# joshuacwnewton/swiftwatcher

Measured on AMD Instinct MI355X. Metric: frames/sec (segment+classify) on 1080p ROI batches, higher is better.
Workload: dtype f64 (image_filtering), f32 (CNN)

## Files before the change

include/swk.h:

```cpp
#ifndef SWK_H
#define SWK_H

#include <stdint.h>

#ifdef __cplusplus
extern "C" {
#endif

#define SWK_ABI_VERSION 2

enum {
    SWK_OK = 0,
    SWK_ERR_ARG = -1,
    SWK_ERR_HIP = -2,
    SWK_ERR_NOGPU = -3,
    SWK_ERR_CAPACITY = -4,
    SWK_ERR_NOMEM = -5,
    SWK_ERR_STALE = -6
};

enum { SWK_MEM_HOST = 0, SWK_MEM_DEVICE = 1 };

enum { SWK_ORDER_RASTER = 0, SWK_ORDER_BLOCK2X2 = 1 };

// ... 106 lines not shown
int32_t swk_regionprops_u8(swk_ctx *ctx, const uint8_t *labels, int32_t count, int32_t H, int32_t W,
                           int32_t seg_cap, swk_segment *segs, int32_t *nseg);

int32_t swk_classifier_input(swk_ctx *ctx, const uint8_t *crops, int64_t crops_bytes, const int64_t *offsets,
                             const int32_t *hw, int32_t nseg, const float mean[3], const float std_[3],
                             uint8_t *patches, float *net, int32_t net_mem);
int32_t swk_classifier_input_window(swk_ctx *ctx, const uint8_t *crops, int64_t crops_bytes, const int64_t *offsets,
                                    const int32_t *hw, int32_t nseg, const float mean[3], const float std_[3],
                                    int32_t pad, int32_t channels_last, uint8_t *patches, float *net, int32_t net_mem);

int32_t swk_segment_inputs(swk_ctx *ctx, const swk_input *in, int32_t frame_h, int32_t frame_w,
                           const swk_segment *segs, const int32_t *nseg, int32_t seg_cap, int32_t min_h, int32_t min_w,
                           const float mean[3], const float std_[3], int32_t pad, int32_t channels_last, int32_t first,
                           int32_t net_cap, float *net, int32_t *seg_frame, int32_t *total, int32_t *skipped);
int32_t swk_segment_inputs_last(swk_ctx *ctx, int32_t min_h, int32_t min_w, const float mean[3], const float std_[3],
                                int32_t pad, int32_t channels_last, int32_t first, int32_t net_cap, float *net,
                                int32_t *seg_frame, int32_t *total, int32_t *skipped);

int32_t swk_nhwc_bias_relu_place(void *stream, const float *src, int32_t n, int32_t sh, int32_t sw, int32_t c, int32_t crop_y,
                                 int32_t crop_x, int32_t h, int32_t w, const float *bias, float *dst, int32_t dH, int32_t dW,
                                 int32_t dC, int32_t off_y, int32_t off_x, int32_t c_off);
int32_t swk_nhwc_maxpool3s2(void *stream, const float *src, int32_t n, int32_t h, int32_t w, int32_t c, float *dst);
int32_t swk_nhwc_head2_relu_mean(void *stream, const float *x, int32_t n, int32_t px, int32_t c, const float *w, const float *bias,
                                 const float *ring, float n_pos, float *out);
int32_t swk_nhwc_head2_dropout_relu_mean(void *stream, const float *x, int32_t n, int32_t px, int32_t c, const int32_t *pos, const float *bg,
                                         int32_t n_pos, const float *w, const float *bias, const uint64_t *keys, uint64_t seed,
                                         int32_t samples, float *out);
int32_t swk_nhwc_conv7x7s2_bias_relu(void *stream, const float *src, int32_t n, int32_t side, int32_t lo, int32_t m, const float *weight,
                                     const float *bias, int32_t cout, float *dst);
int32_t swk_nhwc_conv1x1_bias_relu_place(void *stream, const float *src, int32_t n, int32_t sh, int32_t sw, int32_t cin, int32_t crop_y,
                                         int32_t crop_x, int32_t h, int32_t w, const float *weight, const float *bias, int32_t cout,
                                         float *dst, int32_t dH, int32_t dW, int32_t dC, int32_t off_y, int32_t off_x, int32_t c_off);

int32_t swk_nhwc_maxpool3s2_conv1x1_bias_relu_place(void *stream, const float *src, int32_t n, int32_t t, int32_t cin, const float *weight,
                                                    const float *bias, int32_t cout, float *dst, int32_t dH, int32_t dW, int32_t dC,
                                                    int32_t off_y, int32_t off_x, const float *ring, int32_t live_lo, int32_t live_n);


int32_t swk_nhwc_conv3x3_bias_relu_place(void *stream, const float *src, int32_t n, int32_t t, int32_t cin, const float *weight_t,
                                         const float *bias, int32_t cout, float *dst, int32_t dH, int32_t dW, int32_t dC, int32_t off_y,
                                         int32_t off_x, int32_t c_off);

int32_t swk_winograd_f2x2_3x3_weights(const float *weight, int32_t cout, int32_t cin, float *out);
int32_t swk_nhwc_conv3x3_winograd_bias_relu_place(void *stream, const float *src, int32_t n, int32_t t, int32_t cin, const float *weight_w,
                                                  const float *bias, int32_t cout, float *dst, int32_t dH, int32_t dW, int32_t dC,
                                                  int32_t off_y, int32_t off_x, int32_t c_off);

int32_t swk_winograd_f2x2_3x3_weights_bf16s(const float *weight, int32_t cout, int32_t cin, uint16_t *out);
int32_t swk_nhwc_conv3x3_winograd_bf16s_bias_relu_place(void *stream, const float *src, int32_t n, int32_t t, int32_t cin,
                                                        const uint16_t *weight_s, const float *bias, int32_t cout, float *dst, int32_t dH,
                                                        int32_t dW, int32_t dC, int32_t off_y, int32_t off_x, int32_t c_off);

int32_t swk_track_costs(const double *prev_c, const double *prev_hist0, const uint8_t *prev_has_hist,
                        const double *curr_c, int32_t n_prev, int32_t n_curr, double *cost);
int32_t swk_lsap(const double *cost, int32_t n_rows, int32_t n_cols, int32_t *col4row);

int32_t swk_median_blur_u8(const uint8_t *src, int32_t H, int32_t W, int32_t channels, int32_t ksize, uint8_t *dst);
int32_t swk_otsu_threshold_u8(const uint8_t *src, int64_t count, uint8_t *dst, int32_t *thresh);
int32_t swk_canny_u8(const uint8_t *src, int32_t H, int32_t W, int32_t low, int32_t high, uint8_t *dst);
int32_t swk_dilate_up_u8(const uint8_t *src, int32_t H, int32_t W, int32_t N, uint8_t *dst);
int32_t swk_roi_mask(const uint8_t *frame, int32_t H, int32_t W, int64_t row_stride, const int32_t corners[4],
                     int32_t crop_region[4], uint8_t *mask, int64_t mask_capacity);


#ifdef __cplusplus
}
// ... 3 lines not shown
```

swiftwatcher_amd/_lib.py:

```python
import ctypes
import os
import threading

import numpy as np

_HERE = os.path.dirname(os.path.abspath(__file__))
LIB_PATH = os.environ.get("SWK_LIB", os.path.join(_HERE, "libswk.so"))

ABI_VERSION = 2
MEM_HOST, MEM_DEVICE = 0, 1
ERR_STALE = -6
STAGE_DENSE, STAGE_WHOLE, STAGE_ROWS, STAGE_2D, STAGE_DEVICE = 0, 1, 2, 3, -1
STAGES = ("gray", "rpca", "bilateral", "thresh", "opened", "labels")
ORDER_RASTER, ORDER_BLOCK2X2 = 0, 1
GRAY_Q14, GRAY_Q15 = 0, 1
YUV_I420, YUV_NV12 = 0, 1
K_GRAY, K_IALM_STATS, K_IALM_PASS, K_IALM_SMALL, K_FILTER, K_CCL, K_PROPS, K_COPY = range(8)
KERNEL_FAMILIES = ["gray", "ialm_stats", "ialm_pass", "ialm_small", "filter", "ccl", "props", "copy"]

c_u8p = ctypes.POINTER(ctypes.c_uint8)
c_f64p = ctypes.POINTER(ctypes.c_double)
c_i32p = ctypes.POINTER(ctypes.c_int32)


# ... 66 lines not shown
    "swk_rpca_epilogue": (ctypes.c_int32, [ctypes.c_void_p, ctypes.c_void_p, ctypes.c_int64, ctypes.c_void_p]),
    "swk_bilateral_u8": (ctypes.c_int32, [ctypes.c_void_p, ctypes.c_void_p, ctypes.c_int32, ctypes.c_int32, ctypes.c_int32, ctypes.c_int32, ctypes.c_double, ctypes.c_double, ctypes.c_int32, ctypes.c_void_p]),
    "swk_thresh_tozero_u8": (ctypes.c_int32, [ctypes.c_void_p, ctypes.c_void_p, ctypes.c_int64, ctypes.c_int32, ctypes.c_void_p]),
    "swk_grey_open3x3_u8": (ctypes.c_int32, [ctypes.c_void_p, ctypes.c_void_p, ctypes.c_int32, ctypes.c_int32, ctypes.c_int32, ctypes.c_void_p]),
    "swk_grey_open_u8": (ctypes.c_int32, [ctypes.c_void_p, ctypes.c_void_p] + [ctypes.c_int32] * 5 + [ctypes.c_void_p]),
    "swk_resize_linear_u8": (ctypes.c_int32, [ctypes.c_void_p, ctypes.c_void_p] + [ctypes.c_int32] * 6 + [ctypes.c_void_p]),
    "swk_ccl_u8": (ctypes.c_int32, [ctypes.c_void_p, ctypes.c_void_p, ctypes.c_int32, ctypes.c_int32, ctypes.c_int32, ctypes.c_int32, ctypes.c_int32, ctypes.c_void_p, ctypes.c_void_p]),
    "swk_regionprops_u8": (ctypes.c_int32, [ctypes.c_void_p, ctypes.c_void_p, ctypes.c_int32, ctypes.c_int32, ctypes.c_int32, ctypes.c_int32, ctypes.c_void_p, ctypes.c_void_p]),
    "swk_classifier_input": (ctypes.c_int32, [ctypes.c_void_p, ctypes.c_void_p, ctypes.c_int64, ctypes.c_void_p, ctypes.c_void_p, ctypes.c_int32, ctypes.c_void_p, ctypes.c_void_p, ctypes.c_void_p, ctypes.c_void_p, ctypes.c_int32]),
    "swk_set_sparse_speculation": (ctypes.c_int32, [ctypes.c_void_p, ctypes.c_double]),
    "swk_set_integer_start": (ctypes.c_int32, [ctypes.c_void_p, ctypes.c_int32]),
    "swk_last_integer_start_windows": (ctypes.c_int32, [ctypes.c_void_p, ctypes.c_void_p]),
    "swk_debug_ialm_start": (ctypes.c_int32, [ctypes.c_void_p, ctypes.c_void_p, ctypes.c_int32, ctypes.c_int32, ctypes.c_int32, ctypes.c_double] + [ctypes.c_void_p] * 7),
    "swk_debug_ialm_first_step": (ctypes.c_int32, [ctypes.c_void_p, ctypes.c_void_p, ctypes.c_int32, ctypes.c_int32, ctypes.c_int32, ctypes.c_double] + [ctypes.c_void_p] * 7),
    "swk_last_host_stage": (ctypes.c_int32, [ctypes.c_void_p, ctypes.c_void_p, ctypes.c_int32]),
    "swk_debug_resize_table": (ctypes.c_int32, [ctypes.c_void_p, ctypes.c_int32, ctypes.c_int32, ctypes.c_int32, ctypes.c_void_p, ctypes.c_void_p]),
    "swk_last_eig_sweeps": (ctypes.c_int32, [ctypes.c_void_p, ctypes.c_void_p]),
    "swk_set_norm_speculation": (ctypes.c_int32, [ctypes.c_void_p, ctypes.c_double]),
    "swk_set_norm_guard": (ctypes.c_int32, [ctypes.c_void_p, ctypes.c_double]),
    "swk_prof_guard_windows": (ctypes.c_int32, [ctypes.c_void_p, ctypes.c_void_p]),
    "swk_last_stopping_norms": (ctypes.c_int32, [ctypes.c_void_p, ctypes.c_void_p, ctypes.c_void_p, ctypes.c_int32]),
    "swk_set_start_refine": (ctypes.c_int32, [ctypes.c_void_p, ctypes.c_double]),
    "swk_prof_refined_windows": (ctypes.c_int32, [ctypes.c_void_p, ctypes.c_void_p, ctypes.c_void_p]),
    "swk_prof_pass_bytes_per_element": (ctypes.c_int32, [ctypes.c_void_p, ctypes.c_void_p]),
    "swk_prof_redo_batches": (ctypes.c_int32, [ctypes.c_void_p, ctypes.c_void_p]),
    "swk_prof_redo_windows": (ctypes.c_int32, [ctypes.c_void_p, ctypes.c_void_p]),
    "swk_nhwc_bias_relu_place": (ctypes.c_int32, [ctypes.c_void_p, ctypes.c_void_p] + [ctypes.c_int32] * 8 + [ctypes.c_void_p, ctypes.c_void_p] + [ctypes.c_int32] * 6),
    "swk_set_cnn_tuning": (ctypes.c_int32, [ctypes.c_int32, ctypes.c_int32]),
    "swk_nhwc_conv7x7s2_bias_relu": (ctypes.c_int32, [ctypes.c_void_p, ctypes.c_void_p, ctypes.c_int32, ctypes.c_int32, ctypes.c_int32, ctypes.c_int32, ctypes.c_void_p, ctypes.c_void_p, ctypes.c_int32, ctypes.c_void_p]),
    "swk_nhwc_conv1x1_bias_relu_place": (ctypes.c_int32, [ctypes.c_void_p, ctypes.c_void_p] + [ctypes.c_int32] * 8 + [ctypes.c_void_p, ctypes.c_void_p, ctypes.c_int32, ctypes.c_void_p] + [ctypes.c_int32] * 6),
    "swk_nhwc_conv3x3_bias_relu_place": (ctypes.c_int32, [ctypes.c_void_p, ctypes.c_void_p, ctypes.c_int32, ctypes.c_int32, ctypes.c_int32, ctypes.c_void_p, ctypes.c_void_p, ctypes.c_int32, ctypes.c_void_p] + [ctypes.c_int32] * 6),
    "swk_nhwc_conv3x3_winograd_bias_relu_place": (ctypes.c_int32, [ctypes.c_void_p, ctypes.c_void_p, ctypes.c_int32, ctypes.c_int32, ctypes.c_int32, ctypes.c_void_p, ctypes.c_void_p, ctypes.c_int32, ctypes.c_void_p] + [ctypes.c_int32] * 6),
    "swk_winograd_f2x2_3x3_weights": (ctypes.c_int32, [ctypes.c_void_p, ctypes.c_int32, ctypes.c_int32, ctypes.c_void_p]),
    "swk_nhwc_conv3x3_winograd_bf16s_bias_relu_place": (ctypes.c_int32, [ctypes.c_void_p, ctypes.c_void_p, ctypes.c_int32, ctypes.c_int32, ctypes.c_int32, ctypes.c_void_p, ctypes.c_void_p, ctypes.c_int32, ctypes.c_void_p] + [ctypes.c_int32] * 6),
    "swk_winograd_f2x2_3x3_weights_bf16s": (ctypes.c_int32, [ctypes.c_void_p, ctypes.c_int32, ctypes.c_int32, ctypes.c_void_p]),
    "swk_nhwc_maxpool3s2_conv1x1_bias_relu_place": (ctypes.c_int32, [ctypes.c_void_p, ctypes.c_void_p, ctypes.c_int32, ctypes.c_int32, ctypes.c_int32, ctypes.c_void_p, ctypes.c_void_p, ctypes.c_int32, ctypes.c_void_p] + [ctypes.c_int32] * 5 + [ctypes.c_void_p, ctypes.c_int32, ctypes.c_int32]),
    "swk_nhwc_maxpool3s2": (ctypes.c_int32, [ctypes.c_void_p, ctypes.c_void_p, ctypes.c_int32, ctypes.c_int32, ctypes.c_int32, ctypes.c_int32, ctypes.c_void_p]),
    "swk_nhwc_head2_relu_mean": (ctypes.c_int32, [ctypes.c_void_p, ctypes.c_void_p, ctypes.c_int32, ctypes.c_int32, ctypes.c_int32, ctypes.c_void_p,
                                                  ctypes.c_void_p, ctypes.c_void_p, ctypes.c_float, ctypes.c_void_p]),
    "swk_nhwc_head2_dropout_relu_mean": (ctypes.c_int32, [ctypes.c_void_p, ctypes.c_void_p, ctypes.c_int32, ctypes.c_int32, ctypes.c_int32, ctypes.c_void_p,
                                                          ctypes.c_void_p, ctypes.c_int32, ctypes.c_void_p, ctypes.c_void_p, ctypes.c_void_p, ctypes.c_uint64,
                                                          ctypes.c_int32, ctypes.c_void_p]),
    "swk_segment_inputs": (ctypes.c_int32, [ctypes.c_void_p, ctypes.c_void_p, ctypes.c_int32, ctypes.c_int32, ctypes.c_void_p, ctypes.c_void_p, ctypes.c_int32, ctypes.c_int32, ctypes.c_int32, ctypes.c_void_p, ctypes.c_void_p, ctypes.c_int32, ctypes.c_int32, ctypes.c_int32, ctypes.c_int32, ctypes.c_void_p, ctypes.c_void_p, ctypes.c_void_p, ctypes.c_void_p]),
    "swk_segment_inputs_last": (ctypes.c_int32, [ctypes.c_void_p, ctypes.c_int32, ctypes.c_int32, ctypes.c_void_p, ctypes.c_void_p, ctypes.c_int32, ctypes.c_int32, ctypes.c_int32, ctypes.c_int32, ctypes.c_void_p, ctypes.c_void_p, ctypes.c_void_p, ctypes.c_void_p]),
    "swk_device_alloc": (ctypes.c_int32, [ctypes.c_void_p, ctypes.c_int64, ctypes.POINTER(ctypes.c_void_p)]),
    "swk_device_free": (ctypes.c_int32, [ctypes.c_void_p, ctypes.c_void_p]),
    "swk_device_read": (ctypes.c_int32, [ctypes.c_void_p, ctypes.c_void_p, ctypes.c_void_p, ctypes.c_int64]),
    "swk_classifier_input_window": (ctypes.c_int32, [ctypes.c_void_p, ctypes.c_void_p, ctypes.c_int64, ctypes.c_void_p, ctypes.c_void_p, ctypes.c_int32, ctypes.c_void_p, ctypes.c_void_p, ctypes.c_int32, ctypes.c_int32, ctypes.c_void_p, ctypes.c_void_p, ctypes.c_int32]),
    "swk_track_costs": (ctypes.c_int32, [ctypes.c_void_p, ctypes.c_void_p, ctypes.c_void_p, ctypes.c_void_p, ctypes.c_int32, ctypes.c_int32, ctypes.c_void_p]),
    "swk_lsap": (ctypes.c_int32, [ctypes.c_void_p, ctypes.c_int32, ctypes.c_int32, ctypes.c_void_p]),
    "swk_median_blur_u8": (ctypes.c_int32, [ctypes.c_void_p, ctypes.c_int32, ctypes.c_int32, ctypes.c_int32, ctypes.c_int32, ctypes.c_void_p]),
    "swk_otsu_threshold_u8": (ctypes.c_int32, [ctypes.c_void_p, ctypes.c_int64, ctypes.c_void_p, ctypes.c_void_p]),
    "swk_canny_u8": (ctypes.c_int32, [ctypes.c_void_p, ctypes.c_int32, ctypes.c_int32, ctypes.c_int32, ctypes.c_int32, ctypes.c_void_p]),
    "swk_dilate_up_u8": (ctypes.c_int32, [ctypes.c_void_p, ctypes.c_int32, ctypes.c_int32, ctypes.c_int32, ctypes.c_void_p]),
    "swk_roi_mask": (ctypes.c_int32, [ctypes.c_void_p, ctypes.c_int32, ctypes.c_int32, ctypes.c_int64, ctypes.c_void_p, ctypes.c_void_p, ctypes.c_void_p, ctypes.c_int64]),
    "swk_pinned_alloc": (ctypes.c_int32, [ctypes.c_int32, ctypes.c_int64, ctypes.POINTER(ctypes.c_void_p)]),
    "swk_pinned_free": (ctypes.c_int32, [ctypes.c_void_p]),
    "swk_cut_boxes": (ctypes.c_int32, [ctypes.c_void_p, ctypes.c_int32, ctypes.c_int64, ctypes.c_int32, ctypes.c_int32, ctypes.c_void_p, ctypes.c_void_p, ctypes.c_void_p, ctypes.c_void_p]),
    "swk_stage_frames": (ctypes.c_int32, [ctypes.c_void_p, ctypes.c_int32, ctypes.c_int64, ctypes.c_int32, ctypes.c_int32, ctypes.c_int64, ctypes.c_int64, ctypes.c_void_p, ctypes.c_int32]),
    "swk_prof_enable": (ctypes.c_int32, [ctypes.c_void_p, ctypes.c_int32]),
    "swk_prof_reset": (ctypes.c_int32, [ctypes.c_void_p]),
    "swk_prof_get": (ctypes.c_int32, [ctypes.c_void_p, ctypes.c_int32, ctypes.POINTER(ctypes.c_double), ctypes.POINTER(ctypes.c_int64)]),
    "swk_prof_window_iters": (ctypes.c_int32, [ctypes.c_void_p, ctypes.POINTER(ctypes.c_int64)]),
    "swk_set_ialm_variant": (ctypes.c_int32, [ctypes.c_void_p, ctypes.c_int32]),
    "swk_set_pass_tuning": (ctypes.c_int32, [ctypes.c_void_p, ctypes.c_int32]),
    "swk_set_eig_method": (ctypes.c_int32, [ctypes.c_void_p, ctypes.c_int32]),
# ... 721 lines not shown
```

swiftwatcher_amd/csrc/build.py:

```python
import os
import subprocess
import sys

HERE = os.path.dirname(os.path.abspath(__file__))
PKG = os.path.dirname(HERE)
ROOT = os.path.dirname(PKG)
LIB = os.path.join(PKG, "libswk.so")
SOURCES = ["swk_api.hip", "ialm.hip", "ialm_mfma.hip", "ialm_mstate.hip", "ialm_small.hip", "ialm_refine.hip", "ialm_gram8.hip", "groups.hip", "filters.hip", "yuv.hip", "ccl.hip", "classify_input.hip", "cnn_aux.hip", "cnn_conv1.hip", "cnn_conv1x1.hip", "cnn_expand_bf16.hip", "cnn_conv3x3.hip", "cnn_wino3x3.hip", "cnn_wino3x3_bf16s.hip", "cnn_poolsq.hip", "tracker.cpp", "roi_mask.cpp", "host_stage.cpp"]
HEADERS = ["swk_internal.h", "cnn_common.h", "ialm_small_dev.h", os.path.join(ROOT, "include", "swk.h"), os.path.join(ROOT, "include", "swk_debug.h")]
FLAGS = ["--offload-arch=gfx950", "-O3", "-std=c++17", "-fPIC", "-ffp-contract=off",
         "-fvisibility=hidden", "-Wall", "-Wno-unused-function", "-I", os.path.join(ROOT, "include"), "-I", HERE]


def _stale(out, deps):
    if not os.path.exists(out):
        return True
    t = os.path.getmtime(out)
    return any(os.path.getmtime(d) > t for d in deps)


def build(force=False, verbose=False):
    hipcc = os.environ.get("HIPCC", "/opt/rocm/bin/hipcc")
    objdir = os.path.join(HERE, "build")
    os.makedirs(objdir, exist_ok=True)
    hdrs = [h if os.path.isabs(h) else os.path.join(HERE, h) for h in HEADERS]
    objs = []
    procs = []
    for src in SOURCES:
        sp = os.path.join(HERE, src)
        obj = os.path.join(objdir, src + ".o")
        objs.append(obj)
        if force or _stale(obj, [sp] + hdrs + [os.path.abspath(__file__)]):
            cmd = [hipcc] + FLAGS + ["-c", sp, "-o", obj]
            if verbose:
                print(" ".join(cmd))
            procs.append((src, subprocess.Popen(cmd)))
    for src, p in procs:
        if p.wait() != 0:
            raise RuntimeError("hipcc failed on " + src)
    if force or procs or _stale(LIB, objs):
        cmd = [hipcc, "--offload-arch=gfx950", "-shared", "-fPIC", "-pthread", "-o", LIB] + objs
# ... 9 lines not shown
```

swiftwatcher_amd/csrc/cnn_common.h:

```cpp
#pragma once
#include "swk_internal.h"

#include <cstring>

namespace swk {

typedef float f16v __attribute__((ext_vector_type(16)));
typedef __bf16 bf16x8 __attribute__((ext_vector_type(8)));

struct Place {
    float *dst;
    int dH, dW, dC, off_y, off_x, c_off;
};
struct Crop {
    int sh, sw, crop_y, crop_x;
};

inline bool place_ok(const Place &p, int h, int w, int c, bool quads, const Crop *crop = nullptr)
{
    if (!p.dst || c < 1 || p.off_y < 0 || p.off_x < 0 || p.off_y + h > p.dH || p.off_x + w > p.dW || p.c_off < 0 || p.c_off + c > p.dC) return false;
    if (quads && ((c & 3) || (p.dC & 3) || (p.c_off & 3) || ((uintptr_t)p.dst & 15))) return false;
    return !crop || (crop->crop_y >= 0 && crop->crop_x >= 0 && crop->crop_y + h <= crop->sh && crop->crop_x + w <= crop->sw);
}

int launch_expand1x1_split_bf16(hipStream_t s, const float *src, int64_t rows, const Crop &cr, int cin, int h, int w, const float *wgt,
                                const float *bias, int cout, const Place &pl);
extern int g_expand_split_bf16;
extern int g_wino_bf16s_layout;

__device__ __forceinline__ void store_bias_relu(float *q, const f16v &acc, int g, const float4 b)
{
    float4 v;
    v.x = fmaxf(acc[4 * g] + b.x, 0.0f);
    v.y = fmaxf(acc[4 * g + 1] + b.y, 0.0f);
    v.z = fmaxf(acc[4 * g + 2] + b.z, 0.0f);
    v.w = fmaxf(acc[4 * g + 3] + b.w, 0.0f);
    *(float4 *)q = v;
}

__device__ __forceinline__ void split3(float x, __bf16 &a, __bf16 &b, __bf16 &c)
{
    a = (__bf16)x;
    const float r = x - (float)a;
    b = (__bf16)r;
    c = (__bf16)(r - (float)b);
}
inline void split3_host(float x, uint16_t part[3])
{
    for (int i = 0; i < 3; ++i) {
        uint32_t u;
        float back;
        memcpy(&u, &x, 4);
        u = (u + 0x7fffu + ((u >> 16) & 1u)) & 0xffff0000u;
        memcpy(&back, &u, 4);
        part[i] = (uint16_t)(u >> 16);
        x -= back;
    }
}

inline void winograd_U(const float g[9], double U[4][4])
// ... 31 lines not shown
```

swiftwatcher_amd/csrc/cnn_conv1x1.hip:

```cpp
#include "cnn_common.h"

namespace swk {

template <int NBLK, int KC, int D, int CS, int NWV>
__global__ __launch_bounds__(64 * NWV) void k_conv1x1_relu_place(const float *__restrict__ src, int64_t rows, int sh, int sw, int cin, int crop_y,
                                                            int crop_x, int h, int w, const float *__restrict__ wgt, const float *__restrict__ bias,
                                                            int cout, float *__restrict__ dst, int dH, int dW, int dC, int off_y, int off_x, int c_off,
                                                            FastDiv fhw, FastDiv fw)
{
    constexpr int NP = 32 * NBLK, PITCH = NP + 1, KH = KC / 2, NV = KH / 4, NB = NBLK / CS, NT = 64 * NWV, SLOTS = NWV / CS;
    static_assert(NBLK % CS == 0 && NWV % CS == 0, "column splits");
    extern __shared__ float lds[];
    const int tid = threadIdx.x, lane = tid & 63, wave = tid >> 6, r = lane & 31, hh = lane >> 5;
    float *lbias = lds + ((cin * PITCH + 3) & ~3);
    const int hw = h * w;
    const int cs = wave % CS;
    const int64_t ntiles = (rows + 31) >> 5, stride = (int64_t)gridDim.x * SLOTS;
    int64_t tile = (int64_t)blockIdx.x * SLOTS + wave / CS;

    auto locate = [&](int64_t t, int64_t &ro) -> const float * {
        const unsigned m = (unsigned)t * 32u + (unsigned)r;
        const bool valid = m < (unsigned)rows;
        const unsigned mm = valid ? m : (unsigned)rows - 1u;
        const unsigned b = fhw.div(mm), rem = mm - b * (unsigned)hw;
// ... 140 lines not shown

int32_t swk_nhwc_conv1x1_bias_relu_place(void *stream, const float *src, int32_t n, int32_t sh, int32_t sw, int32_t cin, int32_t crop_y,
                                         int32_t crop_x, int32_t h, int32_t w, const float *weight, const float *bias, int32_t cout,
                                         float *dst, int32_t dH, int32_t dW, int32_t dC, int32_t off_y, int32_t off_x, int32_t c_off)
{
    const swk::Place pl{dst, dH, dW, dC, off_y, off_x, c_off};
    const swk::Crop cr{sh, sw, crop_y, crop_x};
    if (!src || !weight || !bias || n < 1 || h < 1 || w < 1 || cin < 16 || (cin & 15) || cin > 1024 || cout > 256 ||
        !swk::place_ok(pl, h, w, cout, true, &cr) || ((((uintptr_t)src) | ((uintptr_t)weight)) & 15))
        return SWK_ERR_ARG;
    using namespace swk;
    const int64_t rows = (int64_t)n * h * w;
    hipStream_t s = (hipStream_t)stream;
    if (g_expand_split_bf16 && cout == 4 * cin) {
        const int rc = launch_expand1x1_split_bf16(s, src, rows, cr, cin, h, w, weight, bias, cout, pl);
        if (rc != SWK_ERR_ARG) return rc;
    }
    switch ((cout + 31) / 32) {
    case 1: return launch_conv1x1<1>(s, src, rows, cr, cin, h, w, weight, bias, cout, pl);
    case 2: return launch_conv1x1<2>(s, src, rows, cr, cin, h, w, weight, bias, cout, pl);
    case 3: return launch_conv1x1<3>(s, src, rows, cr, cin, h, w, weight, bias, cout, pl);
    case 4: return launch_conv1x1<4>(s, src, rows, cr, cin, h, w, weight, bias, cout, pl);
    case 6: return launch_conv1x1<6>(s, src, rows, cr, cin, h, w, weight, bias, cout, pl);
    case 8: return launch_conv1x1<8>(s, src, rows, cr, cin, h, w, weight, bias, cout, pl);
    default: return SWK_ERR_ARG;
    }
}

int32_t swk_set_cnn_tuning(int32_t knob, int32_t value)
{
    if (knob == 0 && (value == 0 || value == 1)) { swk::g_conv1x1_ring = value; return SWK_OK; }
    if (knob == 1 && (value == 0 || value == 1)) { swk::g_expand_split_bf16 = value; return SWK_OK; }
    if (knob == 2 && value >= 0 && value <= 2) { swk::g_wino_bf16s_layout = value; return SWK_OK; }
    return SWK_ERR_ARG;
}

}
#pragma GCC visibility pop
```

swiftwatcher_amd/segment_classification.py:

```python
import ctypes
import os
import threading

import numpy as np
import torch
from torch import nn

IMAGENET_MEAN = (0.485, 0.456, 0.406)
IMAGENET_STD = (0.229, 0.224, 0.225)
RESIZE = 24
PAD = (224 - 24) // 2


class Fire(nn.Module):

    def __init__(self, inplanes, squeeze_planes, expand1x1_planes, expand3x3_planes):
        super().__init__()
        self.squeeze = nn.Conv2d(inplanes, squeeze_planes, kernel_size=1)
        self.squeeze_activation = nn.ReLU(inplace=True)
        self.expand1x1 = nn.Conv2d(squeeze_planes, expand1x1_planes, kernel_size=1)
        self.expand1x1_activation = nn.ReLU(inplace=True)
        self.expand3x3 = nn.Conv2d(squeeze_planes, expand3x3_planes, kernel_size=3, padding=1)
        self.expand3x3_activation = nn.ReLU(inplace=True)

# ... 98 lines not shown
                lo, hi, size = a, b, out_size
        self.final = (lo, hi, size)
        self.final_bg = x[:, :, lo:hi + 1, lo:hi + 1].contiguous()
        ring = head.clone()
        ring[:, :, lo:hi + 1, lo:hi + 1] = 0
        self.ring_sum = ring.sum(dim=(2, 3))
        self.n_pos = float(size * size)
        self.head_bg = x.permute(0, 2, 3, 1).reshape(size * size, x.shape[1]).contiguous()
        self.head_pos = torch.tensor([r * size + c for r in range(lo, hi + 1) for c in range(lo, hi + 1)], dtype=torch.int32, device=dev)
        self.sq_bg = []
        with torch.no_grad():
            for kind, layer, tile, off, n, pad, crop in self.plan:
                if kind != "fire":
                    self.sq_bg.append(None)
                    continue
                sq = layer.squeeze_activation(layer.squeeze(tile))
                if pad[0] or pad[1]:
                    sq = torch.nn.functional.pad(sq, (pad[0], pad[1], pad[0], pad[1]))
                self.sq_bg.append(sq.contiguous())
        self._cap = 0
        self._buf = None
        self.memory_format = torch.channels_last if dev.type == "cuda" else torch.contiguous_format
        if self.memory_format == torch.channels_last:
            model.to(memory_format=torch.channels_last)
        self.own_kernels = os.environ.get("SWK_OWN_CNN_KERNELS", "1") == "1"
        self._head = None
        self.winograd = True
        self.wino_split_bf16 = os.environ.get("SWK_WINO_SPLIT_BF16", "1") == "1"
        self.fuse_pool = os.environ.get("SWK_FUSE_POOL", "1") == "1"
        self._w1 = None
        self._wt3 = {}
        self._ww3 = {}
        self._ws3 = {}

    def macs_per_segment(self):
        m = self.model
        c1 = m.features[0]
        side = (self.IN_HI - self.IN_LO + 1 - 7) // 2 + 1
        executed = useful = side * side * c1.out_channels * c1.in_channels * 49
        last_n = None
        on_gpu = self.ring_sum.is_cuda and self.memory_format == torch.channels_last and self.own_kernels
        for kind, layer, tile, off, n, pad, crop in self.plan:
            if kind != "fire":
                continue
            t = tile.shape[2] + pad[0] + pad[1]
            sq, e1, e3 = layer.squeeze, layer.expand1x1, layer.expand3x3
            executed += n * n * sq.out_channels * sq.in_channels
            e1_side = n if on_gpu else t
            executed += e1_side * e1_side * e1.out_channels * e1.in_channels
            wino = on_gpu and self.winograd and e3.out_channels == 4 * e3.in_channels and e3.in_channels in (16, 32, 48, 64)
            if wino:
                tiles = ((t - 2 + 1) // 2) ** 2
                executed += tiles * 16 * e3.out_channels * e3.in_channels
            else:
                executed += (t - 2) ** 2 * e3.out_channels * e3.in_channels * 9
            useful += n * n * sq.out_channels * sq.in_channels
            useful += crop[1] ** 2 * (e1.out_channels * e1.in_channels + e3.out_channels * e3.in_channels * 9)
            last_n = crop[1]
        head = m.classifier[1]
        executed += last_n * last_n * head.out_channels * head.in_channels
        useful += last_n * last_n * head.out_channels * head.in_channels
        return int(executed), int(useful)

    def _buffers(self, batch):
        if batch <= self._cap:
            return self._buf
# ... 7 lines not shown
        for j, (kind, layer, tile, off, n, pad, crop) in enumerate(self.plan):
            nxt = self.plan[j + 1][0] if j + 1 < len(self.plan) else "head"
            if kind == "fire" and nxt != "pool":
                if nxt == "fire":
                    _, _, ntile, noff, nn, _, _ = self.plan[j + 1]
                    bg = ntile[:, :, noff:noff + nn, noff:noff + nn]
                else:
                    bg = self.final_bg
                assert bg.shape[2] == crop[1] and bg.shape[1] == layer.expand1x1.out_channels + layer.expand3x3.out_channels
                live.append(bg.expand(batch, -1, -1, -1).contiguous(memory_format=self.memory_format))
            else:
                live.append(None)
        self._buf, self._cap = (bufs, live), batch
        self.version = getattr(self, "version", 0) + 1
        return self._buf

    def _gpu_path(self, tiles):
        return tiles.is_cuda and self.memory_format == torch.channels_last and all(
            kind != "fire" or not (pad[0] or pad[1]) for kind, _, _, _, _, pad, _ in self.plan)

    def reserve(self, batch):
        self._buffers(batch)
        if self.ring_sum.is_cuda:
            self._aux_buffers(batch)
            self._prepare_operands()

    def _prepare_operands(self):
        if not (self.own_kernels and self.ring_sum.is_cuda and self.memory_format == torch.channels_last):
            return
        self._conv1_operand()
        for j, (kind, layer, tile, off, n, pad, crop) in enumerate(self.plan):
            if kind == "fire":
                self._w3_operand(j, layer.expand3x3)
        self._head_operand()

    def _conv1_operand(self):
        if self._w1 is None:
            self._w1 = self.model.features[0].weight.detach().contiguous(memory_format=torch.contiguous_format).clone()
        return self._w1

    def _head_operand(self):
        if self._head is None:
            head = self.model.classifier[1]
            self._head = (head.weight.detach().reshape(head.out_channels, -1).contiguous(), head.bias.detach().contiguous(),
                          self.ring_sum.reshape(-1).contiguous())
        return self._head

    def _w3_kind(self, conv):
        cin, cout = conv.in_channels, conv.out_channels
        if self.winograd and cout == 4 * cin and cin in (16, 32, 48, 64):
            return "bf16s" if self.wino_split_bf16 and cin != 16 else "f32"
        return "direct"

    def _w3_operand(self, j, conv, kind=None):
        from . import _lib
        kind = kind or self._w3_kind(conv)
        cache = {"bf16s": self._ws3, "f32": self._ww3, "direct": self._wt3}[kind]
        w = cache.get(j)
        if w is not None:
            return w
        cin, cout = conv.in_channels, conv.out_channels
        dev = conv.weight.device
        if kind == "direct":
            w = conv.weight.detach().permute(2, 3, 1, 0).contiguous(memory_format=torch.contiguous_format)
        else:
            lib = _lib.load()
            wc = conv.weight.detach().to("cpu", torch.float32).contiguous()
            ncol = 32 * (-(-cout // 32))
            if kind == "bf16s":
                out = torch.empty(3 * 16 * cin * ncol, dtype=torch.int16)
                if lib.swk_winograd_f2x2_3x3_weights_bf16s(wc.data_ptr(), cout, cin, out.data_ptr()):
                    raise RuntimeError("swk_winograd_f2x2_3x3_weights_bf16s failed")
            else:
                out = torch.empty(16 * cin * ncol, dtype=torch.float32)
                if lib.swk_winograd_f2x2_3x3_weights(wc.data_ptr(), cout, cin, out.data_ptr()):
                    raise RuntimeError("swk_winograd_f2x2_3x3_weights failed")
            w = out.to(dev)
        cache[j] = w
        return w
# ... 30 lines not shown
            else:
                _, _, _, poff, pn, _, _ = self.plan[j + 1]
                assert pn == cn
                dest = bufs[j + 1][:k, :, poff:poff + pn, poff:poff + pn]
            cp = c + pad[0]
            torch.clamp_min(e1[:, :, cp:cp + cn, cp:cp + cn], 0, out=dest[:, :c1])
            torch.clamp_min(e3, 0, out=dest[:, c1:])
            x = dest
        s = torch.relu(m.classifier[1](x)).sum(dim=(2, 3))
        return (s + self.ring_sum) / self.n_pos

    def _forward_hip_glue(self, tiles, row0=0, dropout=None):
        from . import _lib
        lib = _lib.load()
        stream = ctypes.c_void_p(torch.cuda.current_stream(tiles.device).cuda_stream)
        m = self.model
        conv2d = torch.nn.functional.conv2d
        k = tiles.shape[0]
        bufs, live = self._buffers(row0 + k)
        rows = slice(row0, row0 + k)
        cl = torch.channels_last

        def nhwc(t):
            return t if t.is_contiguous(memory_format=cl) else t.contiguous(memory_format=cl)

        def place(e, bias, dest, crop, size, off, c_off):
            e = nhwc(e)
            rc = lib.swk_nhwc_bias_relu_place(stream, e.data_ptr(), k, e.shape[2], e.shape[3], e.shape[1], crop, crop, size, size,
                                              bias.data_ptr(), dest.data_ptr(), dest.shape[2], dest.shape[3], dest.shape[1],
                                              off, off, c_off)
            if rc:
                raise RuntimeError("swk_nhwc_bias_relu_place failed (%d)" % rc)

        def conv1x1(src, crop, size, conv, dest, off, c_off):
            src = nhwc(src)
            wgt = conv.weight.reshape(conv.out_channels, conv.in_channels)
            rc = lib.swk_nhwc_conv1x1_bias_relu_place(stream, src.data_ptr(), k, src.shape[2], src.shape[3], src.shape[1], crop, crop,
                                                      size, size, wgt.data_ptr(), conv.bias.data_ptr(), conv.out_channels,
                                                      dest.data_ptr(), dest.shape[2], dest.shape[3], dest.shape[1], off, off, c_off)
            if rc:
                raise RuntimeError("swk_nhwc_conv1x1_bias_relu_place failed (%d)" % rc)

        def conv3x3(src, j, conv, dest, off, c_off):
            src = nhwc(src)
            cin, cout = conv.in_channels, conv.out_channels
            kind = self._w3_kind(conv)
            if kind != "direct" and k * src.shape[2] * src.shape[2] * cin * 4 < (1 << 32):
                ww = self._w3_operand(j, conv, kind)
                fn = "swk_nhwc_conv3x3_winograd_bf16s_bias_relu_place" if kind == "bf16s" else "swk_nhwc_conv3x3_winograd_bias_relu_place"
                rc = getattr(lib, fn)(stream, src.data_ptr(), k, src.shape[2], cin, ww.data_ptr(), conv.bias.data_ptr(), cout,
                                      dest.data_ptr(), dest.shape[2], dest.shape[3], dest.shape[1], off, off, c_off)
                if rc:
                    raise RuntimeError("%s failed (%d)" % (fn, rc))
                return
            wt = self._w3_operand(j, conv, "direct")
            assert src.shape[2] == src.shape[3]
            rc = lib.swk_nhwc_conv3x3_bias_relu_place(stream, src.data_ptr(), k, src.shape[2], src.shape[1], wt.data_ptr(),
                                                      conv.bias.data_ptr(), conv.out_channels, dest.data_ptr(), dest.shape[2],
                                                      dest.shape[3], dest.shape[1], off, off, c_off)
            if rc:
                raise RuntimeError("swk_nhwc_conv3x3_bias_relu_place failed (%d)" % rc)

        def pool(src, dst):
            rc = lib.swk_nhwc_maxpool3s2(stream, src.data_ptr(), k, src.shape[2], src.shape[3], src.shape[1], dst.data_ptr())
            if rc:
                raise RuntimeError("swk_nhwc_maxpool3s2 failed (%d)" % rc)

        def pool_squeeze(src, conv, dest, off, ring=None, live=(0, 0)):
            wgt = conv.weight.reshape(conv.out_channels, conv.in_channels)
# ... 18 lines not shown
                raise RuntimeError("swk_nhwc_conv7x7s2_bias_relu failed (%d)" % rc)
        else:
            e = conv2d(nhwc(tiles), conv1.weight, None, stride=conv1.stride)
            place(e, conv1.bias, c1buf, a, b - a, 0, 0)
        fuse = self.fuse_pool and self.own_kernels
        to_pool = c1buf
        pool_ring, pool_live = None, (0, 0)
        x = aux["pool_in"][rows]
        if not fuse:
            pool(c1buf, x)
        pi = 0
        for j, (kind, layer, tile, off, n, pad, crop) in enumerate(self.plan):
            if kind == "pool":
                x = aux["pool_out"][pi][rows]
                if fuse:
                    to_pool, pool_ring, pool_live = bufs[j][rows], bufs[j][0:1], (off, n)
                else:
                    pool(bufs[j][rows], x)
                pi += 1
                continue
            sq = bufs[j][rows]
            c, cn = crop
            c1 = layer.expand1x1.out_channels
            if live[j] is not None:
                dest, doff = live[j][rows], 0
            else:
                dest, doff = bufs[j + 1][rows], self.plan[j + 1][3]
            if self.own_kernels:
                if fuse and to_pool is not None:
                    assert (to_pool.shape[2] - 3) // 2 + 1 == n
                    pool_squeeze(to_pool, layer.squeeze, sq, off, pool_ring, pool_live)
                    to_pool = None
                else:
                    conv1x1(x, 0, n, layer.squeeze, sq, off, 0)
                conv1x1(sq, off, n, layer.expand1x1, dest, doff + off - c, 0)
            else:
                place(conv2d(x, layer.squeeze.weight, None), layer.squeeze.bias, sq, 0, n, off, 0)
                e1 = conv2d(sq, layer.expand1x1.weight, None)
                place(e1, layer.expand1x1.bias, dest, c, cn, doff, 0)
            if self.own_kernels:
                conv3x3(sq, j, layer.expand3x3, dest, doff, c1)
            else:
                place(conv2d(sq, layer.expand3x3.weight, None), layer.expand3x3.bias, dest, 0, cn, doff, c1)
            x = dest
        head = m.classifier[1]
        if dropout is not None:
            if not (self.own_kernels and head.out_channels == 2 and x.shape[1] in (256, 512, 768, 1024)):
                raise RuntimeError("dropout sampling runs on the library's HIP head kernel (own kernels, a two-class head)")
            hw, hb, _ = self._head_operand()
            keys, seed, samples = dropout
            return _dropout_head(x, self.head_pos, self.head_bg, int(self.n_pos), hw, hb, keys, seed, samples)
        if self.own_kernels and head.out_channels == 2 and x.shape[1] in (256, 512, 768, 1024) and x.is_contiguous(memory_format=cl):
            hw, hb, ring = self._head_operand()
            out = torch.empty((k, 2), dtype=torch.float32, device=x.device)
            rc = lib.swk_nhwc_head2_relu_mean(stream, x.data_ptr(), k, x.shape[2] * x.shape[3], x.shape[1], hw.data_ptr(), hb.data_ptr(),
                                              ring.data_ptr(), self.n_pos, out.data_ptr())
            if rc:
                raise RuntimeError("swk_nhwc_head2_relu_mean failed (%d)" % rc)
            return out
        px = x.permute(0, 2, 3, 1).reshape(-1, x.shape[1])
        s = torch.relu(torch.nn.functional.linear(px, head.weight.view(head.out_channels, -1), head.bias))
        s = s.view(k, -1, head.out_channels).sum(dim=1)
        return (s + self.ring_sum) / self.n_pos

    def _aux_buffers(self, batch):
        if getattr(self, "_aux_cap", 0) >= batch:
            return self._aux
# ... 356 lines not shown
```

Measured before the change: 42960.

## Add split-bf16 MFMA squeeze 1x1 conv kernel for large-cin fire layers

Adds a new HIP kernel that computes the squeeze 1x1 convolution for specific (cin, cout) shapes by splitting fp32 activations and weights into three bf16 parts each and accumulating six bf16 MFMA products. Weights are pre-split on the host into a lane-ordered layout and streamed into double-buffered LDS via DMA, overlapping with activation loads. The Python model routes non-fused squeeze convs through it when a pre-split operand exists. This trades six MFMA ops per product for near-fp32 accuracy, replacing a slower fp32 path, and adds host-side weight preparation and extra LDS pressure.

```diff
diff --git a/include/swk.h b/include/swk.h
--- a/include/swk.h
+++ b/include/swk.h
@@ -162,6 +162,13 @@
                                          int32_t crop_x, int32_t h, int32_t w, const float *weight, const float *bias, int32_t cout,
                                          float *dst, int32_t dH, int32_t dW, int32_t dC, int32_t off_y, int32_t off_x, int32_t c_off);
 
+int32_t swk_conv1x1_bf16s_route(int32_t cin, int32_t cout);
+int32_t swk_conv1x1_weights_bf16s(const float *weight, int32_t cout, int32_t cin, uint16_t *out);
+int32_t swk_nhwc_conv1x1_bf16s_bias_relu_place(void *stream, const float *src, int32_t n, int32_t sh, int32_t sw, int32_t cin, int32_t crop_y,
+                                               int32_t crop_x, int32_t h, int32_t w, const float *weight, const uint16_t *weight_s,
+                                               const float *bias, int32_t cout, float *dst, int32_t dH, int32_t dW, int32_t dC, int32_t off_y,
+                                               int32_t off_x, int32_t c_off);
+
 int32_t swk_nhwc_maxpool3s2_conv1x1_bias_relu_place(void *stream, const float *src, int32_t n, int32_t t, int32_t cin, const float *weight,
                                                     const float *bias, int32_t cout, float *dst, int32_t dH, int32_t dW, int32_t dC,
                                                     int32_t off_y, int32_t off_x, const float *ring, int32_t live_lo, int32_t live_n);
diff --git a/swiftwatcher_amd/_lib.py b/swiftwatcher_amd/_lib.py
--- a/swiftwatcher_amd/_lib.py
+++ b/swiftwatcher_amd/_lib.py
@@ -122,6 +122,9 @@
     "swk_nhwc_conv3x3_bias_relu_place": (ctypes.c_int32, [ctypes.c_void_p, ctypes.c_void_p, ctypes.c_int32, ctypes.c_int32, ctypes.c_int32, ctypes.c_void_p, ctypes.c_void_p, ctypes.c_int32, ctypes.c_void_p] + [ctypes.c_int32] * 6),
     "swk_nhwc_conv3x3_winograd_bias_relu_place": (ctypes.c_int32, [ctypes.c_void_p, ctypes.c_void_p, ctypes.c_int32, ctypes.c_int32, ctypes.c_int32, ctypes.c_void_p, ctypes.c_void_p, ctypes.c_int32, ctypes.c_void_p] + [ctypes.c_int32] * 6),
     "swk_winograd_f2x2_3x3_weights": (ctypes.c_int32, [ctypes.c_void_p, ctypes.c_int32, ctypes.c_int32, ctypes.c_void_p]),
+    "swk_conv1x1_bf16s_route": (ctypes.c_int32, [ctypes.c_int32, ctypes.c_int32]),
+    "swk_conv1x1_weights_bf16s": (ctypes.c_int32, [ctypes.c_void_p, ctypes.c_int32, ctypes.c_int32, ctypes.c_void_p]),
+    "swk_nhwc_conv1x1_bf16s_bias_relu_place": (ctypes.c_int32, [ctypes.c_void_p, ctypes.c_void_p] + [ctypes.c_int32] * 8 + [ctypes.c_void_p, ctypes.c_void_p, ctypes.c_void_p, ctypes.c_int32, ctypes.c_void_p] + [ctypes.c_int32] * 6),
     "swk_nhwc_conv3x3_winograd_bf16s_bias_relu_place": (ctypes.c_int32, [ctypes.c_void_p, ctypes.c_void_p, ctypes.c_int32, ctypes.c_int32, ctypes.c_int32, ctypes.c_void_p, ctypes.c_void_p, ctypes.c_int32, ctypes.c_void_p] + [ctypes.c_int32] * 6),
     "swk_winograd_f2x2_3x3_weights_bf16s": (ctypes.c_int32, [ctypes.c_void_p, ctypes.c_int32, ctypes.c_int32, ctypes.c_void_p]),
     "swk_nhwc_maxpool3s2_conv1x1_bias_relu_place": (ctypes.c_int32, [ctypes.c_void_p, ctypes.c_void_p, ctypes.c_int32, ctypes.c_int32, ctypes.c_int32, ctypes.c_void_p, ctypes.c_void_p, ctypes.c_int32, ctypes.c_void_p] + [ctypes.c_int32] * 5 + [ctypes.c_void_p, ctypes.c_int32, ctypes.c_int32]),
diff --git a/swiftwatcher_amd/csrc/build.py b/swiftwatcher_amd/csrc/build.py
--- a/swiftwatcher_amd/csrc/build.py
+++ b/swiftwatcher_amd/csrc/build.py
@@ -6,7 +6,7 @@
 PKG = os.path.dirname(HERE)
 ROOT = os.path.dirname(PKG)
 LIB = os.path.join(PKG, "libswk.so")
-SOURCES = ["swk_api.hip", "ialm.hip", "ialm_mfma.hip", "ialm_mstate.hip", "ialm_small.hip", "ialm_refine.hip", "ialm_gram8.hip", "groups.hip", "filters.hip", "yuv.hip", "ccl.hip", "classify_input.hip", "cnn_aux.hip", "cnn_conv1.hip", "cnn_conv1x1.hip", "cnn_expand_bf16.hip", "cnn_conv3x3.hip", "cnn_wino3x3.hip", "cnn_wino3x3_bf16s.hip", "cnn_poolsq.hip", "tracker.cpp", "roi_mask.cpp", "host_stage.cpp"]
+SOURCES = ["swk_api.hip", "ialm.hip", "ialm_mfma.hip", "ialm_mstate.hip", "ialm_small.hip", "ialm_refine.hip", "ialm_gram8.hip", "groups.hip", "filters.hip", "yuv.hip", "ccl.hip", "classify_input.hip", "cnn_aux.hip", "cnn_conv1.hip", "cnn_conv1x1.hip", "cnn_expand_bf16.hip", "cnn_squeeze_bf16s.hip", "cnn_conv3x3.hip", "cnn_wino3x3.hip", "cnn_wino3x3_bf16s.hip", "cnn_poolsq.hip", "tracker.cpp", "roi_mask.cpp", "host_stage.cpp"]
 HEADERS = ["swk_internal.h", "cnn_common.h", "ialm_small_dev.h", os.path.join(ROOT, "include", "swk.h"), os.path.join(ROOT, "include", "swk_debug.h")]
 FLAGS = ["--offload-arch=gfx950", "-O3", "-std=c++17", "-fPIC", "-ffp-contract=off",
          "-fvisibility=hidden", "-Wall", "-Wno-unused-function", "-I", os.path.join(ROOT, "include"), "-I", HERE]
diff --git a/swiftwatcher_amd/csrc/cnn_common.h b/swiftwatcher_amd/csrc/cnn_common.h
--- a/swiftwatcher_amd/csrc/cnn_common.h
+++ b/swiftwatcher_amd/csrc/cnn_common.h
@@ -26,6 +26,7 @@
 int launch_expand1x1_split_bf16(hipStream_t s, const float *src, int64_t rows, const Crop &cr, int cin, int h, int w, const float *wgt,
                                 const float *bias, int cout, const Place &pl);
 extern int g_expand_split_bf16;
+extern int g_squeeze_bf16s;
 extern int g_wino_bf16s_layout;
 
 __device__ __forceinline__ void store_bias_relu(float *q, const f16v &acc, int g, const float4 b)
diff --git a/swiftwatcher_amd/csrc/cnn_conv1x1.hip b/swiftwatcher_amd/csrc/cnn_conv1x1.hip
--- a/swiftwatcher_amd/csrc/cnn_conv1x1.hip
+++ b/swiftwatcher_amd/csrc/cnn_conv1x1.hip
@@ -196,6 +196,7 @@
     if (knob == 0 && (value == 0 || value == 1)) { swk::g_conv1x1_ring = value; return SWK_OK; }
     if (knob == 1 && (value == 0 || value == 1)) { swk::g_expand_split_bf16 = value; return SWK_OK; }
     if (knob == 2 && value >= 0 && value <= 2) { swk::g_wino_bf16s_layout = value; return SWK_OK; }
+    if (knob == 4 && value >= 0 && value <= 2) { swk::g_squeeze_bf16s = value; return SWK_OK; }
     return SWK_ERR_ARG;
 }
 
diff --git a/swiftwatcher_amd/csrc/cnn_squeeze_bf16s.hip b/swiftwatcher_amd/csrc/cnn_squeeze_bf16s.hip
--- /dev/null
+++ b/swiftwatcher_amd/csrc/cnn_squeeze_bf16s.hip
@@ -0,0 +1,223 @@
+#include "cnn_common.h"
+
+namespace swk {
+
+__device__ __forceinline__ void split3x8(const float4 lo, const float4 hi, bf16x8 &p1, bf16x8 &p2, bf16x8 &p3)
+{
+    const float v[8] = {lo.x, lo.y, lo.z, lo.w, hi.x, hi.y, hi.z, hi.w};
+#pragma unroll
+    for (int j = 0; j < 8; ++j) {
+        __bf16 a, b, c;
+        split3(v[j], a, b, c);
+        p1[j] = a; p2[j] = b; p3[j] = c;
+    }
+}
+
+constexpr int SQ_NBLK = 2;
+constexpr int SQ_CHUNK_STEPS = 4;
+constexpr int SQ_PIECES = SQ_CHUNK_STEPS * SQ_NBLK * 3;
+constexpr int SQ_CHUNK_BYTES = SQ_PIECES * 1024;
+
+template <int NCH, int NWV>
+__global__ __launch_bounds__(64 * NWV, NWV == 8 ? 4 : 3) void k_squeeze_bf16s_relu_place(const float *__restrict__ src, int64_t rows, int sh, int sw, int crop_y,
+                                                                  int crop_x, int h, int w, const uint16_t *__restrict__ ws,
+                                                                  const float *__restrict__ bias, int cout, float *__restrict__ dst, int dH,
+                                                                  int dW, int dC, int off_y, int off_x, int c_off, FastDiv fhw, FastDiv fw)
+{
+    constexpr int CIN = 64 * NCH, NP = 32 * SQ_NBLK, PW = SQ_PIECES / NWV;
+    static_assert(SQ_PIECES % NWV == 0 && PW % 3 == 0, "whole copy statements per wave");
+    extern __shared__ uint4 lds_q[];
+    float *lbias = (float *)(lds_q + 2 * SQ_PIECES * 64);
+    const int tid = threadIdx.x, lane = tid & 63, wave = __builtin_amdgcn_readfirstlane(tid >> 6), r = lane & 31, hh = lane >> 5;
+    const int hw = h * w;
+    const int64_t ntiles = (rows + 31) >> 5, stride = (int64_t)gridDim.x * NWV;
+    int64_t tbase = (int64_t)blockIdx.x * NWV;
+
+    auto locate = [&](int64_t t, unsigned &b, unsigned &y, unsigned &x) -> bool {
+        const int64_t m64 = t * 32 + r;
+        const bool valid = m64 < rows;
+        const unsigned mm = valid ? (unsigned)m64 : (unsigned)rows - 1u;
+        b = fhw.div(mm);
+        const unsigned rem = mm - b * (unsigned)hw;
+        y = fw.div(rem);
+        x = rem - y * (unsigned)w;
+        return valid;
+    };
+    auto source = [&](int64_t t) -> const float * {
+        unsigned b, y, x;
+        locate(t, b, y, x);
+        return src + (((int64_t)b * sh + crop_y + y) * sw + crop_x + x) * (int64_t)CIN + 16 * hh;
+    };
+    const unsigned wvoff = (unsigned)(lane * 16);
+    auto w_issue = [&](int c, int buf, unsigned voff) {
+        const char *gp = (const char *)ws + (int64_t)c * SQ_CHUNK_BYTES + wave * (PW * 1024);
+        const unsigned l = __builtin_amdgcn_readfirstlane((unsigned)(uintptr_t)((char *)lds_q + buf * SQ_CHUNK_BYTES + wave * (PW * 1024)));
+#pragma unroll
+        for (int i = 0; i < PW; i += 3) lds_dma_copy<3>(l + i * 1024u, gp + i * 1024, voff);
+    };
+
+    if (tbase >= ntiles) return;
+    float4 raw[2][4];
+    w_issue(0, 0, wvoff);
+    const float *q = source(tbase + wave);
+#pragma unroll
+    for (int t = 0; t < 2; ++t)
+#pragma unroll
+        for (int v = 0; v < 4; ++v) raw[t][v] = *(const float4 *)(q + 32 * t + 4 * v);
+    for (int i = tid; i < NP; i += 64 * NWV) lbias[i] = i < cout ? bias[i] : 0.0f;
+
+    static_assert(NCH % 2 == 0, "every tile starts in buffer 0");
+    for (; tbase < ntiles; tbase += stride) {
+        const bool more = tbase + stride < ntiles;
+        f16v acc[SQ_NBLK];
+#pragma unroll
+        for (int nb = 0; nb < SQ_NBLK; ++nb)
+#pragma unroll
+            for (int e = 0; e < 16; ++e) acc[nb][e] = 0.0f;
+#pragma unroll 1
+        for (int c = 0; c < NCH; ++c) {
+            lds_dma_wait<4>();
+            __syncthreads();
+            const bool last = c + 1 == NCH;
+            const int buf = c & 1;
+            if (!last) q += 64;
+            else if (more) q = source(tbase + stride + wave);
+            const uint4 *wb = lds_q + buf * (SQ_PIECES * 64) + lane;
+            bf16x8 wq[2][3];
+            auto read_w = [&](int s, int nb, int set) {
+                const uint4 *a = wb + ((s * SQ_NBLK + nb) * 3) * 64;
+                wq[set][0] = __builtin_bit_cast(bf16x8, a[0]); wq[set][1] = __builtin_bit_cast(bf16x8, a[64]); wq[set][2] = __builtin_bit_cast(bf16x8, a[128]);
+            };
+            read_w(0, 0, 0);
+#pragma unroll
+            for (int s = 0; s < SQ_CHUNK_STEPS; ++s) {
+                const int t = s >> 1, u = s & 1;
+                bf16x8 x1, x2, x3;
+                split3x8(raw[t][2 * u], raw[t][2 * u + 1], x1, x2, x3);
+                if (s == 2) {
+                    const uint4 x3w = __builtin_bit_cast(uint4, x3);
+                    unsigned vo = wvoff;
+                    asm volatile("" : "+v"(vo) : "v"(x3w.x), "v"(x3w.y), "v"(x3w.z), "v"(x3w.w));
+                    w_issue(last ? 0 : c + 1, buf ^ 1, vo);
+                }
+                if (u == 1) {
+                    const uint4 x3w = __builtin_bit_cast(uint4, x3);
+                    unsigned qo = 32 * t;
+                    asm volatile("" : "+v"(qo) : "v"(x3w.x), "v"(x3w.y), "v"(x3w.z), "v"(x3w.w));
+#pragma unroll
+                    for (int v = 0; v < 4; ++v) raw[t][v] = *(const float4 *)(q + qo + 4 * v);
+                }
+#pragma unroll
+                for (int nb = 0; nb < SQ_NBLK; ++nb) {
+                    const int i = s * SQ_NBLK + nb, set = i & 1;
+                    if (i + 1 < SQ_CHUNK_STEPS * SQ_NBLK) read_w((i + 1) / SQ_NBLK, (i + 1) % SQ_NBLK, set ^ 1);
+                    acc[nb] = __builtin_amdgcn_mfma_f32_32x32x16_bf16(wq[set][0], x3, acc[nb], 0, 0, 0);
+                    acc[nb] = __builtin_amdgcn_mfma_f32_32x32x16_bf16(wq[set][1], x2, acc[nb], 0, 0, 0);
+                    acc[nb] = __builtin_amdgcn_mfma_f32_32x32x16_bf16(wq[set][2], x1, acc[nb], 0, 0, 0);
+                    acc[nb] = __builtin_amdgcn_mfma_f32_32x32x16_bf16(wq[set][0], x2, acc[nb], 0, 0, 0);
+                    acc[nb] = __builtin_amdgcn_mfma_f32_32x32x16_bf16(wq[set][1], x1, acc[nb], 0, 0, 0);
+                    acc[nb] = __builtin_amdgcn_mfma_f32_32x32x16_bf16(wq[set][0], x1, acc[nb], 0, 0, 0);
+                    if (i + 1 < SQ_CHUNK_STEPS * SQ_NBLK) __builtin_amdgcn_sched_group_barrier(0x100 , 3, 0);
+                    if (u == 1 && nb == 0) __builtin_amdgcn_sched_group_barrier(0x020 , 4, 0);
+                    __builtin_amdgcn_sched_group_barrier(0x008 , 6, 0);
+                }
+            }
+        }
+        unsigned b, y, x;
+        if (locate(tbase + wave, b, y, x)) {
+            float *o = dst + (((int64_t)b * dH + off_y + y) * dW + off_x + x) * (int64_t)dC + c_off + 4 * hh;
+#pragma unroll
+            for (int nb = 0; nb < SQ_NBLK; ++nb)
+#pragma unroll
+                for (int g = 0; g < 4; ++g) {
+                    const int c = nb * 32 + 8 * g;
+                    if (c + 4 * hh < cout) store_bias_relu(o + c, acc[nb], g, *(const float4 *)(lbias + c + 4 * hh));
+                }
+        }
+    }
+    lds_dma_wait<0>();
+}
+
+template <int NCH, int NWV>
+static int launch_squeeze_bf16s_d(hipStream_t s, const float *src, int64_t rows, const Crop &cr, int h, int w, const uint16_t *ws, const float *bias,
+                                  int cout, const Place &pl)
+{
+    constexpr size_t lds = (size_t)2 * SQ_CHUNK_BYTES + 32 * SQ_NBLK * sizeof(float);
+    constexpr int per_cu = 16 / NWV < 3 ? 16 / NWV : 3;
+    static_assert(per_cu >= 2 && per_cu * lds <= 160 * 1024 - 256, "two workgroups per CU");
+    static unsigned long long attr_mask = 0;
+    if (!ensure_dyn_lds((const void *)k_squeeze_bf16s_relu_place<NCH, NWV>, 160 * 1024 - 256, attr_mask)) return SWK_ERR_HIP;
+    if (rows > (int64_t)0x7fffff00) return SWK_ERR_CAPACITY;
+    const int64_t ntiles = (rows + 31) / 32;
+    int64_t blocks = (ntiles + NWV - 1) / NWV;
+    if (blocks > 256 * per_cu) blocks = 256 * per_cu;
+    hipLaunchKernelGGL((k_squeeze_bf16s_relu_place<NCH, NWV>), dim3((unsigned)blocks), dim3(64 * NWV), lds, s, src, rows, cr.sh, cr.sw, cr.crop_y,
+                       cr.crop_x, h, w, ws, bias, cout, pl.dst, pl.dH, pl.dW, pl.dC, pl.off_y, pl.off_x, pl.c_off, FastDiv((unsigned)(h * w)),
+                       FastDiv((unsigned)w));
+    return hipGetLastError() == hipSuccess ? SWK_OK : SWK_ERR_HIP;
+}
+
+template <int NCH>
+static int launch_squeeze_bf16s(hipStream_t s, const float *src, int64_t rows, const Crop &cr, int h, int w, const uint16_t *ws, const float *bias,
+                                int cout, const Place &pl)
+{
+    const int64_t ntiles = (rows + 31) / 32;
+    if (ntiles >= 8 * 256) return launch_squeeze_bf16s_d<NCH, 8>(s, src, rows, cr, h, w, ws, bias, cout, pl);
+    return launch_squeeze_bf16s_d<NCH, 4>(s, src, rows, cr, h, w, ws, bias, cout, pl);
+}
+
+static int squeeze_bf16s_route(int cin, int cout)
+{
+    if (cin == 384 && cout == 64) return 2;
+    if (cin == 384 && cout == 48) return 2;
+    if (cin == 256 && cout == 48) return 2;
+    return 0;
+}
+
+int g_squeeze_bf16s = 0;
+
+}
+
+#pragma GCC visibility push(default)
+extern "C" {
+
+int32_t swk_conv1x1_bf16s_route(int32_t cin, int32_t cout) { return swk::squeeze_bf16s_route(cin, cout); }
+
+int32_t swk_conv1x1_weights_bf16s(const float *weight, int32_t cout, int32_t cin, uint16_t *out)
+{
+    if (!weight || !out || cout < 1 || cin < 64 || (cin & 63)) return SWK_ERR_ARG;
+    const int CG = (cout + 31) / 32;
+    for (int64_t i = 0, e = (int64_t)3 * cin * CG * 32; i < e; ++i) out[i] = 0;
+    for (int co = 0; co < cout; ++co)
+        for (int ci = 0; ci < cin; ++ci) {
+            const int s = 2 * (ci >> 5) + ((ci >> 3) & 1), lane = ((ci >> 4) & 1) * 32 + (co & 31), j = ci & 7, cb = co >> 5;
+            uint16_t part[3];
+            swk::split3_host(weight[(int64_t)co * cin + ci], part);
+            for (int k = 0; k < 3; ++k) out[((((int64_t)s * CG + cb) * 3 + k) * 64 + lane) * 8 + j] = part[k];
+        }
+    return SWK_OK;
+}
+
+int32_t swk_nhwc_conv1x1_bf16s_bias_relu_place(void *stream, const float *src, int32_t n, int32_t sh, int32_t sw, int32_t cin, int32_t crop_y,
+                                               int32_t crop_x, int32_t h, int32_t w, const float *weight, const uint16_t *weight_s,
+                                               const float *bias, int32_t cout, float *dst, int32_t dH, int32_t dW, int32_t dC, int32_t off_y,
+                                               int32_t off_x, int32_t c_off)
+{
+    using namespace swk;
+    const Place pl{dst, dH, dW, dC, off_y, off_x, c_off};
+    const Crop cr{sh, sw, crop_y, crop_x};
+    const int route = squeeze_bf16s_route(cin, cout);
+    if (!route) return SWK_ERR_ARG;
+    if (g_squeeze_bf16s == 1 || (g_squeeze_bf16s == 0 && route != 2))
+        return swk_nhwc_conv1x1_bias_relu_place(stream, src, n, sh, sw, cin, crop_y, crop_x, h, w, weight, bias, cout, dst, dH, dW, dC, off_y,
+                                                off_x, c_off);
+    if (!src || !weight_s || !bias || n < 1 || h < 1 || w < 1 || !place_ok(pl, h, w, cout, true, &cr) || (((uintptr_t)src | (uintptr_t)weight_s) & 15))
+        return SWK_ERR_ARG;
+    const int64_t rows = (int64_t)n * h * w;
+    hipStream_t s = (hipStream_t)stream;
+    if (cin == 256) return launch_squeeze_bf16s<4>(s, src, rows, cr, h, w, weight_s, bias, cout, pl);
+    return launch_squeeze_bf16s<6>(s, src, rows, cr, h, w, weight_s, bias, cout, pl);
+}
+
+}
+#pragma GCC visibility pop
diff --git a/swiftwatcher_amd/segment_classification.py b/swiftwatcher_amd/segment_classification.py
--- a/swiftwatcher_amd/segment_classification.py
+++ b/swiftwatcher_amd/segment_classification.py
@@ -154,6 +154,7 @@
         self._wt3 = {}
         self._ww3 = {}
         self._ws3 = {}
+        self._wsq = {}
 
     def macs_per_segment(self):
         m = self.model
@@ -227,6 +228,7 @@
         for j, (kind, layer, tile, off, n, pad, crop) in enumerate(self.plan):
             if kind == "fire":
                 self._w3_operand(j, layer.expand3x3)
+                self._sq_operand(j, layer.squeeze)
         self._head_operand()
 
     def _conv1_operand(self):
@@ -240,6 +242,22 @@
             self._head = (head.weight.detach().reshape(head.out_channels, -1).contiguous(), head.bias.detach().contiguous(),
                           self.ring_sum.reshape(-1).contiguous())
         return self._head
+
+    def _sq_operand(self, j, conv):
+        from . import _lib
+        if j in self._wsq:
+            return self._wsq[j]
+        lib = _lib.load()
+        cin, cout = conv.in_channels, conv.out_channels
+        w = None
+        if lib.swk_conv1x1_bf16s_route(cin, cout):
+            wc = conv.weight.detach().to("cpu", torch.float32).reshape(cout, cin).contiguous()
+            out = torch.empty(3 * cin * 32 * (-(-cout // 32)), dtype=torch.int16)
+            if lib.swk_conv1x1_weights_bf16s(wc.data_ptr(), cout, cin, out.data_ptr()):
+                raise RuntimeError("swk_conv1x1_weights_bf16s failed")
+            w = out.to(conv.weight.device)
+        self._wsq[j] = w
+        return w
 
     def _w3_kind(self, conv):
         cin, cout = conv.in_channels, conv.out_channels
@@ -336,9 +354,17 @@
             if rc:
                 raise RuntimeError("swk_nhwc_bias_relu_place failed (%d)" % rc)
 
-        def conv1x1(src, crop, size, conv, dest, off, c_off):
+        def conv1x1(src, crop, size, conv, dest, off, c_off, split=None):
             src = nhwc(src)
             wgt = conv.weight.reshape(conv.out_channels, conv.in_channels)
+            if split is not None:
+                rc = lib.swk_nhwc_conv1x1_bf16s_bias_relu_place(stream, src.data_ptr(), k, src.shape[2], src.shape[3], src.shape[1], crop, crop,
+                                                                size, size, wgt.data_ptr(), split.data_ptr(), conv.bias.data_ptr(),
+                                                                conv.out_channels, dest.data_ptr(), dest.shape[2], dest.shape[3],
+                                                                dest.shape[1], off, off, c_off)
+                if rc:
+                    raise RuntimeError("swk_nhwc_conv1x1_bf16s_bias_relu_place failed (%d)" % rc)
+                return
             rc = lib.swk_nhwc_conv1x1_bias_relu_place(stream, src.data_ptr(), k, src.shape[2], src.shape[3], src.shape[1], crop, crop,
                                                       size, size, wgt.data_ptr(), conv.bias.data_ptr(), conv.out_channels,
                                                       dest.data_ptr(), dest.shape[2], dest.shape[3], dest.shape[1], off, off, c_off)
@@ -423,7 +449,7 @@
                     pool_squeeze(to_pool, layer.squeeze, sq, off, pool_ring, pool_live)
                     to_pool = None
                 else:
-                    conv1x1(x, 0, n, layer.squeeze, sq, off, 0)
+                    conv1x1(x, 0, n, layer.squeeze, sq, off, 0, self._sq_operand(j, layer.squeeze))
                 conv1x1(sq, off, n, layer.expand1x1, dest, doff + off - c, 0)
             else:
                 place(conv2d(x, layer.squeeze.weight, None), layer.squeeze.bias, sq, 0, n, off, 0)
```

Result: no change. 43140, median of 5 (+0.4%).
